# OpenBMB/VisRAG

Measured on AMD Instinct MI355X. Metric: page-images embedded/sec (VisRAG-Ret encode, 448x448, bf16 MFMA) + queries/sec@top-10 over 100k-page index, higher is better.
Workload: dtype bf16; 1 GPU; VisRAG-Ret (SigLIP-so400m 26 blk + resampler + MiniCPM-2B 40 layers) bf16 encode batch=32 page images 448x448 per GPU; index 100000 rows x 2304 sharded 1 way(s), 1000 queries top-10; batch_per_gpu=32, global_batch=32, parallelism=dp1 (pages sharded, no data-path collective)

## Files before the change

### include/visrag_hip.h

```cpp
#ifndef VISRAG_HIP_H
#define VISRAG_HIP_H

#include <stddef.h>
#include <stdint.h>

#ifdef __cplusplus
extern "C" {
#endif

#define VR_OK 0
#define VR_ERR_INVALID 1
#define VR_ERR_HIP 2
#define VR_ERR_STATE 3
#define VR_ERR_CAPACITY 4

#define VR_DTYPE_F32 0
#define VR_DTYPE_BF16 1

typedef struct vr_model_s* vr_model_t;
typedef struct vr_index_s* vr_index_t;

typedef struct vr_config {
    int32_t patch_size;
    int32_t vit_dim;
// ... 208 lines not shown

int vr_op_gemm(int device_id, const void* A, int32_t lda, const void* W, int32_t ldw,
               int32_t M, int32_t N, int32_t K, int32_t epilogue, const float* bias,
               const float* resid, float alpha, void* out, int32_t ldo,
               const int32_t* rope_pos, const float* rope_table, int32_t rope_cols,
               int32_t variant, void* stream);
typedef struct vr_gemm_extras {
    const int32_t* rowmap;
    const float* rowbias;
    int32_t rowbias_period, rowbias_ld, rowbias_cols;
    float col_scale;
    int32_t col_scale_n;
    int32_t ksplit;
    int64_t split_stride;
    const int32_t* m_dev;
    int32_t m_sub;
    int32_t raster_gm;
} vr_gemm_extras_t;
int vr_op_gemm_ex(int device_id, const void* A, int32_t lda, const void* W, int32_t ldw,
                  int32_t M, int32_t N, int32_t K, int32_t epilogue, const float* bias,
                  const float* resid, float alpha, void* out, int32_t ldo,
                  const int32_t* rope_pos, const float* rope_table, int32_t rope_cols,
                  int32_t variant, const vr_gemm_extras_t* extras, void* stream);
int vr_op_gemm_warm(int device_id, const void* A, int32_t lda, const void* W, int32_t ldw,
                    int32_t M, int32_t N, int32_t K, int32_t epilogue, const float* bias,
                    const float* resid, float alpha, void* out, int32_t ldo,
                    const int32_t* rope_pos, const float* rope_table, int32_t rope_cols,
                    int32_t variant, const vr_gemm_extras_t* extras, const void* warm, uint64_t warm_bytes, void* stream);
int vr_op_norm(int device_id, int32_t kind, const float* x, int32_t rows, int32_t dim,
               const float* weight, const float* bias, float eps, void* out, int32_t ldo,
               void* stream);
int vr_op_norm_ex(int device_id, int32_t kind, const float* x, int32_t rows, int32_t dim, int32_t ldx, const float* weight,
                  const float* bias, float eps, void* out, int32_t ldo, void* stream);

int vr_op_text_rmsnorm_split(int device_id, const float* x, int32_t rows, int32_t dim, const float* weight, float eps, void* hi,
                             void* lo, void* stream);
int vr_op_text_rope(int device_id, float* qkv, int32_t T, int32_t ld, int32_t rope_cols, const int32_t* pos, const float* table,
                    void* stream);
int vr_op_text_attention(int device_id, const float* qkv, int32_t ld, int32_t E, const int32_t* seq_offsets, int32_t B, int32_t T,
                         int32_t heads, float scale, float* out, void* stream);
int vr_op_text_swiglu_split(int device_id, const float* gu, int32_t T, int32_t ld_gu, int32_t I, int32_t ld_act, void* hi, void* lo,
                            void* stream);
int vr_op_embed_gather(int device_id, const int32_t* ids, int32_t T, const void* table, const void* table_lo, int32_t dim,
                       float scale, float* out, void* stream);
int vr_op_pool(int device_id, const float* h, const int32_t* seq_offsets, int32_t B, int32_t dim, const float* norm_w, float eps,
               float* out, float* tap, int32_t mode, void* stream);
int vr_op_convert(int device_id, int32_t kind, const void* in, void* out, void* out2, int64_t n, int64_t n_total, int32_t* aux,
                  void* stream);
int vr_op_planes_sum(int device_id, const float* parts, int32_t n_parts, int64_t stride, int32_t ldp, int32_t T, int32_t N,
                     float* out, int32_t ldo, float alpha, int32_t accumulate, void* stream);
int vr_op_patch_embed(int device_id, const void* const* imgs, int32_t n, int32_t H, int32_t W, int32_t P, const float* weight,
                      int32_t D, int32_t K, const float* bias, const float* pos, int32_t ld_pos, float* out, int32_t ldo,
                      void* stream);
int vr_op_attention(int device_id, const void* q, int32_t ldq, const void* k, int32_t ldk,
                    const void* v, int32_t ldv, void* out, int32_t ldo,
                    const int32_t* cu_q, const int32_t* cu_kv, int32_t B, int32_t heads,
                    int32_t head_dim, int32_t max_q, int32_t causal, int32_t q_shared,
                    float scale, void* stream);
typedef struct vr_attn_extras {
    int32_t kv_group;
    const int32_t* kv_end;
    const int32_t* q_in_rows;
    int32_t q_head_stride;
    int32_t q_prescaled;
    float* lse;
} vr_attn_extras_t;
int vr_op_attention_ex(int device_id, const void* q, int32_t ldq, const void* k, int32_t ldk,
                       const void* v, int32_t ldv, void* out, int32_t ldo,
                       const int32_t* cu_q, const int32_t* cu_kv, int32_t B, int32_t heads,
                       int32_t head_dim, int32_t max_q, int32_t causal, int32_t q_shared,
                       float scale, const vr_attn_extras_t* extras, void* stream);
int vr_op_attn_combine(int device_id, const void* part, const float* lse, int32_t S, const int32_t* S_dev, int32_t heads,
                       int32_t group, int32_t n_rows, void* out, int32_t ld_out, const void* W, int32_t ldw, int32_t M,
                       int32_t N, int32_t K, int32_t ksplit, int32_t planes, int32_t ldo, int64_t split_stride, void* stream);
int vr_op_gemm_skinny(int device_id, const void* A, int32_t lda, const void* W, int32_t ldw, int32_t M, int32_t N,
                      int32_t K, int32_t ksplit, const float* bias, int32_t swiglu, void* out, int32_t ldo,
                      int64_t split_stride, void* stream);
int vr_op_plane_sum(int device_id, int32_t kind, const float* parts, int32_t nsplit, int64_t split_stride, int32_t ldp,
                    int32_t rows, int32_t dim, float* x, int32_t ldx, float alpha, const float* weight, float eps,
                    void* out, int32_t ldo, void* stream);
int vr_op_chat_attention(int device_id, const void* q, const void* prompt, const void* tails, int32_t layers, int32_t l,
                         int32_t E, int32_t slots, int32_t max_len, int32_t rows, int32_t max_new, int32_t n,
                         const int32_t* step_row, const int32_t* step_slot, const int32_t* step_tail,
                         const int32_t* slot_plen, int32_t force_splits, void* att, void* stream);
int vr_op_chat_select(int device_id, int32_t mode, const float* logits, int32_t ld, int32_t V, const uint32_t* seen,
                      int32_t words, int32_t n_groups, const int32_t* group_offsets, const float* beam_scores, int32_t K,
                      int32_t kout, float repetition_penalty, float temperature, uint64_t seed, int32_t step,
                      float* out_scores, int32_t* out_tokens, int32_t* out_parents, void* stream);
int vr_op_chat_prompt_scatter(int device_id, const void* qkv, int32_t ld, int32_t E, int32_t B, const int32_t* seq_offsets,
                              const int32_t* slots, int32_t n_slots, int32_t max_len, void* kplane, void* vplane, void* stream);

int vr_op_gen_mrope_cache(int device_id, const void* src_bf16, const float* parts, int32_t n_parts, int64_t plane_stride,
                          const float* bias, int32_t ld, int32_t T, int32_t H, int32_t KV, const int32_t* pos3, int32_t pos_stride,
                          int32_t sec_t, int32_t sec_h, const float* inv_freq, void* q_out, int32_t ldq, void* k_cache, void* v_cache,
                          int32_t ld_cache, int32_t cache_row0, const int32_t* row0_dev, const int32_t* cache_rows, int32_t* cu_kv,
                          void* stream);
int vr_op_gen_rope2d(int device_id, void* qkv, int32_t ld, int32_t T, int32_t n_slots, int32_t hh, const int32_t* pos_h,
                     const int32_t* pos_w, int32_t sec_h, const float* freq, void* stream);
int vr_op_gen_sample(int device_id, const float* logits, int32_t vocab, uint32_t* seen, float repetition_penalty, float temperature,
                     uint64_t seed, int32_t step, int32_t* state, int32_t step_from_state, int32_t advance, int32_t* out_token,
                     void* stream);
int vr_op_gen_mark_seen(int device_id, const int32_t* ids, int32_t n, uint32_t* seen, int32_t vocab, void* stream);
int vr_op_gen_decode_begin(int device_id, int32_t* state, int32_t q_rows, void* stream);
int vr_op_gen_rows(int device_id, int32_t kind, const float* src, const int32_t* row_idx, int32_t n, int32_t dim, void* dst,
                   int32_t ld, const void* const* pages, const int32_t* page_w, int32_t n_pages, const int32_t* img, const int32_t* ph,
                   const int32_t* pw, int32_t P, int32_t tp, const float* mean3, const float* std3, void* stream);
// ... 6 lines not shown
```

### visrag_amd/_lib.py

```python
from __future__ import annotations

import ctypes as C
import os
from typing import Optional

_HERE = os.path.dirname(os.path.abspath(__file__))
LIB_PATH = os.path.join(_HERE, "libvisrag_hip.so")

VR_DTYPE_F32, VR_DTYPE_BF16 = 0, 1


class VRConfig(C.Structure):
    _fields_ = [
        ("patch_size", C.c_int32), ("vit_dim", C.c_int32), ("vit_depth", C.c_int32),
        ("vit_heads", C.c_int32), ("vit_hidden", C.c_int32), ("vit_pos_grid", C.c_int32),
        ("vit_ln_eps", C.c_float), ("query_num", C.c_int32), ("resampler_ln_eps", C.c_float),
        ("hidden_size", C.c_int32), ("num_layers", C.c_int32), ("num_heads", C.c_int32),
        ("intermediate_size", C.c_int32), ("vocab_size", C.c_int32), ("rms_norm_eps", C.c_float),
        ("rope_theta", C.c_float), ("scale_emb", C.c_float), ("residual_scale", C.c_float),
        ("max_images", C.c_int32), ("max_patches", C.c_int32), ("max_tokens", C.c_int32),
        ("max_seqs", C.c_int32), ("text_split_precision", C.c_int32),
    ]


# ... 65 lines not shown
    "vr_index_set_search_eps": (C.c_int, [_vp, _f32]),
    "vr_index_search_stats": (C.c_int, [_vp, C.POINTER(_i64), _i32]),
    "vr_index_error_model": (C.c_int, [_vp, C.POINTER(_f32)]),
    "vr_index_search_plan": (C.c_int, [_vp, _i32, C.POINTER(_i32)]),
    "vr_synth_pages": (C.c_int, [C.c_int, _vp, _i32, _i32, _i64, _i64, _vp]),
    "vr_streams_overlap": (C.c_int, [C.c_int, _vp, _vp, C.POINTER(C.c_int32)]),
    "vr_index_set_search_profile": (C.c_int, [_vp, _i32]),
    "vr_index_get_search_profile": (C.c_int, [_vp, C.POINTER(C.c_double), C.POINTER(_i64)]),
    "vr_index_search_keys": (C.c_int, [_vp, _vp, _i32, _i32, _i64, _vp, _i32, _vp]),
    "vr_index_set_groups": (C.c_int, [_vp, C.POINTER(_i64), _i64]),
    "vr_index_search_groups": (C.c_int, [_vp, _vp, _i32, _i32, _vp, _vp, _vp, _i32, _vp]),
    "vr_index_group_search_stats": (C.c_int, [_vp, C.POINTER(_i64), _i32]),
    "vr_index_set_filters": (C.c_int, [_vp, _vp, _i32, _i32, _vp]),
    "vr_index_search_filtered": (C.c_int, [_vp, _vp, _i32, _i32, _vp, _vp, _vp, _i32, _vp]),
    "vr_index_filter_search_stats": (C.c_int, [_vp, C.POINTER(_i64), _i32]),
    "vr_index_search_range": (C.c_int, [_vp, _vp, _i32, _vp, _vp, _i64, _vp, C.POINTER(_i64), _i32, _vp]),
    "vr_index_range_results": (C.c_int, [_vp, _vp, _vp, _i64, _i32, _vp]),
    "vr_index_range_search_stats": (C.c_int, [_vp, C.POINTER(_i64), _i32]),
    "vr_index_rank_rows": (C.c_int, [_vp, _vp, _i32, _vp, _vp, _vp, _vp, _vp, _i32, _vp]),
    "vr_index_count_range": (C.c_int, [_vp, _vp, _i32, _vp, _vp, _i32, _vp, _vp, _i32, _vp]),
    "vr_index_rank_search_stats": (C.c_int, [_vp, C.POINTER(_i64), _i32]),
    "vr_index_search_window": (C.c_int, [_vp, _vp, _i32, _vp, _i32, _vp, _vp, _vp, _i32, _vp]),
    "vr_index_window_search_stats": (C.c_int, [_vp, C.POINTER(_i64), _i32]),
    "vr_index_search_groups_window": (C.c_int, [_vp, _vp, _i32, _vp, _i32, _vp, _vp, _vp, _vp, _i32, _vp]),
    "vr_index_group_window_search_stats": (C.c_int, [_vp, C.POINTER(_i64), _i32]),
    "vr_index_rank_groups": (C.c_int, [_vp, _vp, _i32, _vp, _vp, _vp, _vp, _vp, _vp, _i32, _vp]),
    "vr_index_count_groups_range": (C.c_int, [_vp, _vp, _i32, _vp, _vp, _i32, _vp, _vp, _i32, _vp]),
    "vr_index_group_rank_search_stats": (C.c_int, [_vp, C.POINTER(_i64), _i32]),
    "vr_index_search_multi": (C.c_int, [_vp, _vp, _i32, _vp, _i32, _i32, _i32, _vp, _vp, _vp, _vp, _i32, _vp]),
    "vr_index_multi_search_stats": (C.c_int, [_vp, C.POINTER(_i64), _i32]),
    "vr_index_search_diverse": (C.c_int, [_vp, _vp, _i32, _i32, _i32, _f32, _vp, _vp, _vp, _i32, _vp]),
    "vr_index_remove": (C.c_int, [_vp, C.POINTER(_i64), _i64, C.POINTER(_i64), _vp]),
    "vr_index_update": (C.c_int, [_vp, C.POINTER(_i64), _vp, _i64, _i32, _vp]),
    "vr_index_get_rows": (C.c_int, [_vp, C.POINTER(_i64), _i64, _vp, _vp, _i32, _vp]),
    "vr_topk_merge_keys": (C.c_int, [C.c_int, _vp, _i32, _i32, _i32, _vp, _vp, _vp]),
    "vr_resize_bicubic": (C.c_int, [C.c_int, _vp, _i32, _i32, _i32, _vp, _i32, _i32, _vp]),
    "vr_op_gemm": (C.c_int, [C.c_int, _vp, _i32, _vp, _i32, _i32, _i32, _i32, _i32, _vp, _vp, _f32,
                             _vp, _i32, _vp, _vp, _i32, _i32, _vp]),
    "vr_op_gemm_ex": (C.c_int, [C.c_int, _vp, _i32, _vp, _i32, _i32, _i32, _i32, _i32, _vp, _vp, _f32,
                                _vp, _i32, _vp, _vp, _i32, _i32, C.POINTER(VRGemmExtras), _vp]),
    "vr_op_gemm_warm": (C.c_int, [C.c_int, _vp, _i32, _vp, _i32, _i32, _i32, _i32, _i32, _vp, _vp, _f32,
                                  _vp, _i32, _vp, _vp, _i32, _i32, C.POINTER(VRGemmExtras), _vp, C.c_uint64, _vp]),
    "vr_op_norm": (C.c_int, [C.c_int, _i32, _vp, _i32, _i32, _vp, _vp, _f32, _vp, _i32, _vp]),
    "vr_op_norm_ex": (C.c_int, [C.c_int, _i32, _vp, _i32, _i32, _i32, _vp, _vp, _f32, _vp, _i32, _vp]),
    "vr_op_text_rmsnorm_split": (C.c_int, [C.c_int, _vp, _i32, _i32, _vp, _f32, _vp, _vp, _vp]),
    "vr_op_text_rope": (C.c_int, [C.c_int, _vp, _i32, _i32, _i32, _vp, _vp, _vp]),
    "vr_op_text_attention": (C.c_int, [C.c_int, _vp, _i32, _i32, _vp, _i32, _i32, _i32, _f32, _vp, _vp]),
    "vr_op_text_swiglu_split": (C.c_int, [C.c_int, _vp, _i32, _i32, _i32, _i32, _vp, _vp, _vp]),
    "vr_op_embed_gather": (C.c_int, [C.c_int, _vp, _i32, _vp, _vp, _i32, _f32, _vp, _vp]),
    "vr_op_pool": (C.c_int, [C.c_int, _vp, _vp, _i32, _i32, _vp, _f32, _vp, _vp, _i32, _vp]),
    "vr_op_convert": (C.c_int, [C.c_int, _i32, _vp, _vp, _vp, _i64, _i64, _vp, _vp]),
    "vr_op_planes_sum": (C.c_int, [C.c_int, _vp, _i32, _i64, _i32, _i32, _i32, _vp, _i32, _f32, _i32, _vp]),
    "vr_op_patch_embed": (C.c_int, [C.c_int, C.POINTER(_vp), _i32, _i32, _i32, _i32, _vp, _i32, _i32, _vp, _vp, _i32, _vp, _i32, _vp]),
    "vr_op_attention": (C.c_int, [C.c_int, _vp, _i32, _vp, _i32, _vp, _i32, _vp, _i32, _vp, _vp, _i32,
                                  _i32, _i32, _i32, _i32, _i32, _f32, _vp]),
    "vr_op_attention_ex": (C.c_int, [C.c_int, _vp, _i32, _vp, _i32, _vp, _i32, _vp, _i32, _vp, _vp, _i32,
                                     _i32, _i32, _i32, _i32, _i32, _f32, C.POINTER(VRAttnExtras), _vp]),
    "vr_op_attn_combine": (C.c_int, [C.c_int, _vp, _vp, _i32, _vp, _i32, _i32, _i32, _vp, _i32, _vp, _i32, _i32, _i32, _i32, _i32,
                                     _i32, _i32, _i64, _vp]),
    "vr_op_gemm_skinny": (C.c_int, [C.c_int, _vp, _i32, _vp, _i32, _i32, _i32, _i32, _i32, _vp, _i32, _vp, _i32, _i64, _vp]),
    "vr_op_plane_sum": (C.c_int, [C.c_int, _i32, _vp, _i32, _i64, _i32, _i32, _i32, _vp, _i32, _f32, _vp, _f32, _vp, _i32, _vp]),
    "vr_op_chat_attention": (C.c_int, [C.c_int, _vp, _vp, _vp, _i32, _i32, _i32, _i32, _i32, _i32, _i32, _i32, C.POINTER(_i32),
                                       C.POINTER(_i32), C.POINTER(_i32), C.POINTER(_i32), _i32, _vp, _vp]),
    "vr_op_chat_select": (C.c_int, [C.c_int, _i32, _vp, _i32, _i32, _vp, _i32, _i32, C.POINTER(_i32), C.POINTER(_f32), _i32, _i32,
                                    _f32, _f32, C.c_uint64, _i32, C.POINTER(_f32), C.POINTER(_i32), C.POINTER(_i32), _vp]),
    "vr_op_chat_prompt_scatter": (C.c_int, [C.c_int, _vp, _i32, _i32, _i32, C.POINTER(_i32), C.POINTER(_i32), _i32, _i32, _vp, _vp, _vp]),
    "vr_op_gen_mrope_cache": (C.c_int, [C.c_int, _vp, _vp, _i32, _i64, _vp, _i32, _i32, _i32, _i32, _vp, _i32, _i32, _i32, _vp, _vp, _i32,
                                        _vp, _vp, _i32, _i32, _vp, _vp, _vp, _vp]),
    "vr_op_gen_rope2d": (C.c_int, [C.c_int, _vp, _i32, _i32, _i32, _i32, _vp, _vp, _i32, _vp, _vp]),
    "vr_op_gen_sample": (C.c_int, [C.c_int, _vp, _i32, _vp, _f32, _f32, C.c_uint64, _i32, _vp, _i32, _i32, C.POINTER(_i32), _vp]),
    "vr_op_gen_mark_seen": (C.c_int, [C.c_int, _vp, _i32, _vp, _i32, _vp]),
    "vr_op_gen_decode_begin": (C.c_int, [C.c_int, _vp, _i32, _vp]),
    "vr_op_gen_rows": (C.c_int, [C.c_int, _i32, _vp, _vp, _i32, _i32, _vp, _i32, C.POINTER(_vp), C.POINTER(_i32), _i32, _vp, _vp, _vp,
                                 _i32, _i32, C.POINTER(_f32), C.POINTER(_f32), _vp]),
    "vr_chat_create": (C.c_int, [_vp, C.POINTER(VRChatConfig), C.POINTER(_vp)]),
    "vr_chat_destroy": (C.c_int, [_vp]),
    "vr_chat_load_head": (C.c_int, [_vp, _vp, C.POINTER(_i64), _i32, _i32, _i32]),
    "vr_chat_prefill": (C.c_int, [_vp, _i32, _i32, C.POINTER(_vp), C.POINTER(_i32), _i32, _i32, C.POINTER(_i32), _i32,
                                  C.POINTER(_i32), _vp]),
    "vr_chat_prefill_batch": (C.c_int, [_vp, _i32, C.POINTER(_i32), C.POINTER(_i32), C.POINTER(_vp), C.POINTER(_i32), _i32, _i32,
                                        C.POINTER(_i32), C.POINTER(_i32), C.POINTER(_i32), _vp]),
    "vr_chat_step": (C.c_int, [_vp, _i32, C.POINTER(_i32), C.POINTER(_i32), C.POINTER(_i32), _vp]),
    "vr_chat_select": (C.c_int, [_vp, _i32, _i32, C.POINTER(_i32), C.POINTER(_i32), C.POINTER(_f32), _i32, _f32, _f32, _i32,
                                 C.c_uint64, _i32, C.POINTER(_f32), C.POINTER(_i32), C.POINTER(_i32), _vp]),
    "vr_chat_reorder": (C.c_int, [_vp, _i32, C.POINTER(_i32), C.POINTER(_i32), _vp]),
    "vr_chat_logits": (C.c_int, [_vp, _i32, _vp, _vp]),
    "vr_chat_row_len": (C.c_int, [_vp, _i32, C.POINTER(_i32), C.POINTER(_i32)]),
}
GEN_SIGNATURES = {
    "vg_create": (C.c_int, [C.c_int, C.POINTER(VGConfig), C.POINTER(_vp)]),
    "vg_destroy": (C.c_int, [_vp]),
    "vg_load_weight": (C.c_int, [_vp, C.c_char_p, _vp, C.POINTER(_i64), _i32, _i32, _i32]),
    "vg_finalize": (C.c_int, [_vp]),
    "vg_prefill": (C.c_int, [_vp, _vp, _i32, _vp, _vp, _i32, _vp, _vp]),
    "vg_sample": (C.c_int, [_vp, _f32, _f32, C.c_uint64, _i32, C.POINTER(_i32), _vp]),
    "vg_decode": (C.c_int, [_vp, _i32, C.POINTER(_i32), _vp]),
    "vg_logits": (C.c_int, [_vp, _vp, _vp]),
    "vg_select": (C.c_int, [_vp, _i32]),
    "vg_decode_batch": (C.c_int, [_vp, _i32, C.POINTER(_i32), C.POINTER(_i32), C.POINTER(_i32), _vp]),
    "vg_sample_batch": (C.c_int, [_vp, _i32, C.POINTER(_i32), _f32, _f32, C.c_uint64, _i32, C.POINTER(_i32), _vp]),
    "vg_cache_len": (C.c_int, [_vp, C.POINTER(_i32)]),
    "vg_run_begin": (C.c_int, [_vp, _i32, _f32, _f32, C.c_uint64, _i32, _vp]),
    "vg_run_step": (C.c_int, [_vp]),
    "vg_run_token": (C.c_int, [_vp, _i32, C.POINTER(_i32)]),
    "vg_run_end": (C.c_int, [_vp]),
    "vg_vision_create": (C.c_int, [_vp, C.POINTER(VGVisionConfig)]),
# ... 44 lines not shown
```

### visrag_amd/csrc/encode.hip

```cpp
#include <hip/hip_runtime.h>

#include <algorithm>
#include <cmath>
#include <cstring>
#include <vector>

#include "model.h"

static int run_vision_group(vr_model_s* m, const uint8_t* const* dev_imgs_hostarray, int n, int H, int W,
                            const int32_t* rowmap_host , bool first_group, hipStream_t s) {
    const vr_config_t& c = m->c;
    const int P = c.patch_size, gh = H / P, gw = W / P, N = gh * gw;
    const int D = m->D, Dp = m->Dp, E = m->E, Q = m->Q;
    const int M = n * N;
    GridTables* g = nullptr;
    VRCHK(get_grid(m, gh, gw, &g));

    HIPCHK(hipMemcpyAsync(m->w_imgptr.p, dev_imgs_hostarray, (size_t)n * 8, hipMemcpyHostToDevice, s));
    int* cu = (int*)arena_take(m, (size_t)2 * (n + 1) * 4);
    for (int i = 0; i <= n; ++i) { cu[i] = i * N; cu[n + 1 + i] = i * Q; }
    HIPCHK(hipMemcpyAsync(m->w_cu.p, cu, (size_t)2 * (n + 1) * 4, hipMemcpyHostToDevice, s));
    HIPCHK(hipMemcpyAsync(m->w_rowmap.p, rowmap_host, (size_t)n * Q * 4, hipMemcpyHostToDevice, s));
    const int* cu_tok = m->w_cu.as<int>();
    const int* cu_qry = m->w_cu.as<int>() + (n + 1);

    float* h = m->w_hvit.as<float>();
    {
        GemmArgs a = gemm_args(nullptr, 0, m->patch, M, h, Dp);
        a.rowbias = g->vit_pos.as<float>(); a.rowbias_period = N; a.rowbias_ld = Dp; a.rowbias_cols = Dp;
        HIPCHK(launch_patch_embed((const uint8_t* const*)m->w_imgptr.p, n, H, W, P, a, m->Kpe, s));
    }
    if (first_group) VRCHK(tap_store(m, "vit_embed", h, N, D, Dp, false, s));
    const int ldqkv = pad128(3 * D);
    const int vit_hd = c.vit_dim / c.vit_heads;
    const int vit_qscale_n = D % 64 == 0 ? D : 0;
    const float vit_qscale = (1.0f / sqrtf((float)vit_hd)) * 1.44269504088896340736f;
    for (int l = 0; l < c.vit_depth; ++l) {
        const VitBlock& b = m->blocks[l];
        HIPCHK(launch_layernorm(h, M, D, Dp, b.n1w.v.as<float>(), b.n1b.v.as<float>(), c.vit_ln_eps, m->w_xn.p, Dp, s));
        VRCHK(prof_begin(m, VR_PROF_VIT_QKV, s));
        {
            GemmArgs a = gemm_args(m->w_xn.p, Dp, b.qkv, M, m->w_qkv.p, ldqkv);
            a.col_scale = vit_qscale; a.col_scale_n = vit_qscale_n;
            HIPCHK(launch_gemm(a, EPI_BF16, GEMM_VARIANT_AUTO, s));
        }
        VRCHK(prof_end(m, VR_PROF_VIT_QKV, 2.0 * M * D * 3 * D, s));
        {
            AttnArgs a{};
            a.q = m->w_qkv.p; a.ldq = ldqkv;
            a.k = (const char*)m->w_qkv.p + (size_t)D * 2; a.ldk = ldqkv;
            a.v = (const char*)m->w_qkv.p + (size_t)2 * D * 2; a.ldv = ldqkv;
            a.out = m->w_att.p; a.ldo = Dp; a.cu_q = cu_tok; a.cu_kv = cu_tok; a.B = n; a.heads = c.vit_heads;
            a.head_dim = vit_hd; a.max_q = N; a.causal = 0; a.q_shared = 0; a.scale = 1.0f / sqrtf((float)vit_hd); a.q_prescaled = vit_qscale_n > 0;
            VRCHK(prof_begin(m, VR_PROF_VIT_ATTN, s));
            HIPCHK(launch_attention(a, s));
            VRCHK(prof_end(m, VR_PROF_VIT_ATTN, 4.0 * n * (double)N * N * D, s));
        }
        VRCHK(prof_begin(m, VR_PROF_VIT_PROJ, s));
        {
            GemmArgs a = gemm_args(m->w_att.p, Dp, b.proj, M, h, Dp); a.resid = h;
            HIPCHK(launch_gemm(a, EPI_RESID, GEMM_VARIANT_AUTO, s));
        }
        VRCHK(prof_end(m, VR_PROF_VIT_PROJ, 2.0 * M * D * D, s));
        HIPCHK(launch_layernorm(h, M, D, Dp, b.n2w.v.as<float>(), b.n2b.v.as<float>(), c.vit_ln_eps, m->w_xn.p, Dp, s));
        VRCHK(prof_begin(m, VR_PROF_VIT_FC1, s));
        { GemmArgs a = gemm_args(m->w_xn.p, Dp, b.fc1, M, m->w_mlp.p, m->Fp); HIPCHK(launch_gemm(a, EPI_GELU, GEMM_VARIANT_AUTO, s)); }
        VRCHK(prof_end(m, VR_PROF_VIT_FC1, 2.0 * M * D * m->F, s));
        VRCHK(prof_begin(m, VR_PROF_VIT_FC2, s));
        {
            GemmArgs a = gemm_args(m->w_mlp.p, m->Fp, b.fc2, M, h, Dp); a.resid = h;
            HIPCHK(launch_gemm(a, EPI_RESID, GEMM_VARIANT_AUTO, s));
        }
        VRCHK(prof_end(m, VR_PROF_VIT_FC2, 2.0 * M * D * m->F, s));
        if (l == 0 && first_group) VRCHK(tap_store(m, "vit_block0", h, N, D, Dp, false, s));
    }
    HIPCHK(launch_layernorm(h, M, D, Dp, m->vit_nw.v.as<float>(), m->vit_nb.v.as<float>(), c.vit_ln_eps, m->w_xn.p, Dp, s));
    if (first_group) VRCHK(tap_store(m, "vit_out", m->w_xn.p, N, D, Dp, true, s));

    VRCHK(prof_begin(m, VR_PROF_RESAMPLER, s));
    { GemmArgs a = gemm_args(m->w_xn.p, Dp, m->r_kvproj, M, m->w_kv32.p, E); HIPCHK(launch_gemm(a, EPI_F32, GEMM_VARIANT_AUTO, s)); }
    HIPCHK(launch_layernorm(m->w_kv32.as<float>(), M, E, E, m->r_lnkv_w.v.as<float>(), m->r_lnkv_b.v.as<float>(),
                            c.resampler_ln_eps, m->w_xkv.p, E, s));
    {
// ... 377 lines not shown
```

### visrag_amd/csrc/kernels.h

```cpp
#pragma once
#include <hip/hip_runtime.h>
#include <stdint.h>

#include "gemm_warm.h"

namespace vr {

enum GemmEpilogue { EPI_BF16 = 0, EPI_GELU = 1, EPI_F32 = 2, EPI_RESID = 3, EPI_SWIGLU = 4, EPI_ROPE = 5 };
enum GemmVariant { GEMM_VARIANT_GLDS = 0, GEMM_VARIANT_AUTO = 3, GEMM_VARIANT_192 = 7, GEMM_VARIANT_256IL = 9, GEMM_VARIANT_256W = 12,
                   GEMM_VARIANT_192W = 13, GEMM_VARIANT_128W_192 = 14, GEMM_VARIANT_128W_256 = 15 };

struct GemmArgs {
    const void* A; int lda;
    const void* W; int ldw;
    int M, N, K;
    const float* bias;
    const float* resid;
    float alpha;
    void* out; int ldo;
    const int* rowmap;
    const float* rowbias;
    int rowbias_period, rowbias_ld, rowbias_cols;
    const int* rope_pos;
    const float* rope_table;
// ... 82 lines not shown
hipError_t launch_chat_select(const ChatSel& sel, int mode, const float* logits, int ld, int V, const unsigned* seen, int words, float pen,
                              float temperature, int K, int kout, unsigned long long seed, unsigned step, float* lse,
                              unsigned long long* part, float* o_score, int* o_tok, int* o_par, hipStream_t s);

constexpr int GEN_ATT_SPLITS = 16;
struct GenState {
    int token;
    int pos[3];
    int len;
    int step;
    int splits;
    int pad;
    int cu_q[GEN_ATT_SPLITS + 1], cu_kv[GEN_ATT_SPLITS + 1];
};
struct KvSplit { int splits, chunk; };
__host__ __device__ inline KvSplit gen_kv_split(int L) {
    int splits = min(GEN_ATT_SPLITS, max(1, (L + 127) / 128));
    const int chunk = ((L + splits - 1) / splits + 63) / 64 * 64;
    splits = (L + chunk - 1) / chunk;
    return KvSplit{splits, chunk};
}
struct GenBatch {
    int token[16];
    int pos[3][16];
    int cache_row[16];
    int splits[16];
    int cu_q[16 * GEN_ATT_SPLITS + 1];
    int kv_lo[16 * GEN_ATT_SPLITS], kv_hi[16 * GEN_ATT_SPLITS];
    int q_in[16 * GEN_ATT_SPLITS];
    int sampled[16];
};
hipError_t launch_decode_begin(GenState* st, int q_rows, hipStream_t s);
hipError_t launch_mrope_cache(const void* src_bf16, const float* parts, int n_parts, size_t plane_stride, const float* bias,
                              int ld, int T, int H, int KV, const int* pos3, int pos_stride, int sec_t, int sec_h,
                              const float* inv_freq, void* q_out, int ldq, void* k_cache, void* v_cache, int ld_cache,
                              int cache_row0, int* cu_kv, hipStream_t s, const int* row0_dev = nullptr,
                              const int* cache_rows = nullptr);
hipError_t launch_rope2d_table(const int* pos_h, const int* pos_w, int T, int sec_h, const float* freq, void* cs, hipStream_t s);
hipError_t launch_rope2d_inplace(void* qkv, int ld, int T, int n_slots, int hh, const void* cs, hipStream_t s);
hipError_t launch_mark_seen(const int* ids, int n, unsigned* seen, int vocab, hipStream_t s);
hipError_t launch_sample(const float* logits, int vocab, unsigned* seen, float penalty, float temperature,
                         unsigned long long seed, unsigned step, int* token_out, unsigned long long* scratch64, hipStream_t s,
                         GenState* st = nullptr, int step_from_state = 0, int advance = 0);
hipError_t launch_scatter_rows(const float* src, const int* row_idx, int n, int dim, float* dst, int ld, hipStream_t s);
hipError_t launch_gather_rows_bf16(const float* src, const int* row_idx, int n, int dim, void* dst, int ld, hipStream_t s);
hipError_t launch_patch_rows_u8(const uint8_t* const* pages, const int* page_w, const int* img, const int* ph, const int* pw, int n,
                                int P, int tp, const float* mean3, const float* std3, void* dst, int ld, hipStream_t s);
hipError_t launch_attn_combine(const void* part, const float* lse, int S, int heads, int group, void* out, hipStream_t s,
                               const int* S_dev = nullptr,
                               int n_rows = 1, int ld_out = 0);

hipError_t launch_patch_embed(const uint8_t* const* imgs, int n_imgs, int H, int W, int P, const GemmArgs& g, int Kreal,
                              hipStream_t s);
hipError_t launch_embed_gather(const int* ids, int T, const void* table, int dim, float scale,
                               float* out, hipStream_t s);
hipError_t launch_pool(const float* h, const int* seq_offsets, int B, int dim, const float* norm_w,
                       float eps, float* out, float* tap_hidden, hipStream_t s, int mode = 0);
hipError_t launch_f32_to_bf16(const float* in, void* out, size_t n, hipStream_t s);
hipError_t launch_f32_to_bf16_pad(const float* in, void* out, size_t n, size_t n_total, hipStream_t s,
                                  int* zero_word = nullptr);
hipError_t launch_split_bf16(const float* in, void* hi, void* lo, size_t n, hipStream_t s);
hipError_t launch_iota_pos(const int* seq_offsets, int B, int* pos, hipStream_t s);
hipError_t launch_any_nonzero16(const void* p, size_t n, int* flag, hipStream_t s);

hipError_t launch_rmsnorm_split(const float* x, int rows, int dim, const float* w, float eps, void* hi, void* lo, hipStream_t s);
hipError_t launch_rope_f32(float* qkv, int T, int ld, int rope_cols, const int* pos, const float* table, hipStream_t s);
hipError_t launch_attn_f32(const float* qkv, int ld, int E, const int* seq_of, const int* seq_offsets, int T, int heads,
                           float scale, float* out, hipStream_t s);
hipError_t launch_swiglu_split(const float* gu, int T, int ld_gu, int I, int ld_act, void* hi, void* lo, hipStream_t s);
hipError_t launch_embed_gather_hp(const int* ids, int T, const void* table_hi, const void* table_lo, int dim, float scale,
                                  float* out, hipStream_t s);
hipError_t launch_seq_of(const int* seq_offsets, int B, int* seq_of, hipStream_t s);
hipError_t launch_planes_sum(const float* parts, int n_parts, size_t stride, int ldp, int T, int N, float* out, int ldo, float alpha,
                             bool accumulate, hipStream_t s);

hipError_t launch_synth_pages(uint8_t* out, int n, int size, long long seed, long long first, hipStream_t s);

}
#include <vector>
namespace vr {
int resize_coeffs(int in_size, int out_size, std::vector<int>& bounds, std::vector<int>& kk);
hipError_t launch_resize_h(const uint8_t* in, int in_w, int rows, uint8_t* out, int out_w, const int* bounds,
                           const int* kk, int ksize, hipStream_t s);
hipError_t launch_resize_v(const uint8_t* in, int w, uint8_t* out, int out_h, const int* bounds, const int* kk,
                           int ksize, hipStream_t s);

struct SearchArgs {
    const void* index_bf16;
    const float* index_f32;
    int64_t n_docs;
    int dim;
    const void* q_bf16;
    int convert_q;
    const float* q_f32;
    int nq, k;
    float* cand_scores; int* cand_ids; int n_chunks;
    float* out_scores; int64_t* out_ids;
    float* thr_init;
    int pre_own_chunks;
    float* thr_cert;
    unsigned long long* cand_keys;
    float* score_rows; size_t ld_scores;
    int exact_follows;
    int* huge_seen;
    const float* thr_used;
    float eps_rel;
// ... 195 lines not shown
```

### visrag_amd/csrc/ops.hip

```cpp
#include <hip/hip_runtime.h>

#include <algorithm>
#include <chrono>
#include <map>
#include <tuple>
#include <vector>

#include "engine_common.h"

struct ResizeTab { DevBuf bounds, kk; int ksize = 0; };
static std::map<std::tuple<int, int, int>, ResizeTab> g_resize_tabs;

static int get_resize_tab(int dev, int in_size, int out_size, ResizeTab** out) {
    auto key = std::make_tuple(dev, in_size, out_size);
    auto it = g_resize_tabs.find(key);
    if (it == g_resize_tabs.end()) {
        std::vector<int> b, k;
        ResizeTab t;
        t.ksize = resize_coeffs(in_size, out_size, b, k);
        VRCHK(t.bounds.alloc(b.size() * 4));
        VRCHK(t.kk.alloc(k.size() * 4));
        HIPCHK(hipMemcpy(t.bounds.p, b.data(), b.size() * 4, hipMemcpyHostToDevice));
        HIPCHK(hipMemcpy(t.kk.p, k.data(), k.size() * 4, hipMemcpyHostToDevice));
        it = g_resize_tabs.emplace(key, std::move(t)).first;
// ... 380 lines not shown
    return VR_OK;
}

extern "C" int vr_op_text_swiglu_split(int device_id, const float* gu, int32_t T, int32_t ld_gu, int32_t I, int32_t ld_act, void* hi,
                                       void* lo, void* stream) {
    if (!gu || !hi || !lo) return fail(VR_ERR_INVALID, "NULL argument");
    VRCHK(set_dev(device_id));
    HIPCHK(launch_swiglu_split(gu, T, ld_gu, I, ld_act, hi, lo, (hipStream_t)stream));
    return VR_OK;
}

extern "C" int vr_op_embed_gather(int device_id, const int32_t* ids, int32_t T, const void* table, const void* table_lo, int32_t dim,
                                  float scale, float* out, void* stream) {
    if (!ids || !table || !out) return fail(VR_ERR_INVALID, "NULL argument");
    VRCHK(set_dev(device_id));
    if (!table_lo) HIPCHK(launch_embed_gather(ids, T, table, dim, scale, out, (hipStream_t)stream));
    else HIPCHK(launch_embed_gather_hp(ids, T, table, table_lo, dim, scale, out, (hipStream_t)stream));
    return VR_OK;
}

extern "C" int vr_op_pool(int device_id, const float* h, const int32_t* seq_offsets, int32_t B, int32_t dim, const float* norm_w,
                          float eps, float* out, float* tap, int32_t mode, void* stream) {
    if (!h || !seq_offsets || !norm_w || !out) return fail(VR_ERR_INVALID, "NULL argument");
    VRCHK(set_dev(device_id));
    HIPCHK(launch_pool(h, seq_offsets, B, dim, norm_w, eps, out, tap, (hipStream_t)stream, mode));
    return VR_OK;
}

extern "C" int vr_op_convert(int device_id, int32_t kind, const void* in, void* out, void* out2, int64_t n, int64_t n_total,
                             int32_t* aux, void* stream) {
    if (kind < 0 || kind > 5) return fail(VR_ERR_INVALID, "kind %d: 0 f32->bf16, 1 f32->bf16 + zero pad, 2 hi/lo split, 3 any non-zero, 4 positions, 5 sequence of a token", kind);
    if (!in || (kind != 3 && !out) || (kind == 2 && !out2) || (kind == 3 && !aux)) return fail(VR_ERR_INVALID, "NULL argument");
    VRCHK(set_dev(device_id));
    hipStream_t s = (hipStream_t)stream;
    switch (kind) {
        case 0: HIPCHK(launch_f32_to_bf16((const float*)in, out, (size_t)n, s)); break;
        case 1: HIPCHK(launch_f32_to_bf16_pad((const float*)in, out, (size_t)n, (size_t)n_total, s, aux)); break;
        case 2: HIPCHK(launch_split_bf16((const float*)in, out, out2, (size_t)n, s)); break;
        case 3: HIPCHK(launch_any_nonzero16(in, (size_t)n, aux, s)); break;
        case 4: HIPCHK(launch_iota_pos((const int*)in, (int)n, (int*)out, s)); break;
        default: HIPCHK(launch_seq_of((const int*)in, (int)n, (int*)out, s)); break;
    }
    return VR_OK;
}

extern "C" int vr_op_planes_sum(int device_id, const float* parts, int32_t n_parts, int64_t stride, int32_t ldp, int32_t T, int32_t N,
                                float* out, int32_t ldo, float alpha, int32_t accumulate, void* stream) {
    if (!parts || !out) return fail(VR_ERR_INVALID, "NULL argument");
    VRCHK(set_dev(device_id));
    HIPCHK(launch_planes_sum(parts, n_parts, (size_t)stride, ldp, T, N, out, ldo, alpha, accumulate != 0, (hipStream_t)stream));
    return VR_OK;
}

extern "C" int vr_op_patch_embed(int device_id, const void* const* imgs, int32_t n, int32_t H, int32_t W, int32_t P, const float* weight,
                                 int32_t D, int32_t K, const float* bias, const float* pos, int32_t ld_pos, float* out, int32_t ldo,
                                 void* stream) {
    if (!imgs || !weight || !bias || !pos || !out) return fail(VR_ERR_INVALID, "NULL argument");
    for (int i = 0; i < n; ++i)
        if (!imgs[i]) return fail(VR_ERR_INVALID, "NULL argument");
    VRCHK(set_dev(device_id));
    hipStream_t s = (hipStream_t)stream;
    const int Kreal = 3 * P * P, patches = P > 0 ? (H / P) * (W / P) : 0;
    DevBuf wp, ptrs;
    VRCHK(wp.alloc((size_t)pad256(D > 0 ? D : 1) * (size_t)std::max(std::max(K, Kreal), 1) * 2));
    VRCHK(ptrs.alloc((size_t)(n > 0 ? n : 1) * sizeof(void*)));
    HIPCHK(launch_pack_patch_weight(weight, 0, D, P, wp.p, K, s));
    if (n > 0) HIPCHK(hipMemcpyAsync(ptrs.p, imgs, (size_t)n * sizeof(void*), hipMemcpyHostToDevice, s));
    GemmArgs a{};
    a.W = wp.p; a.ldw = K; a.M = n * patches; a.N = D; a.K = K; a.bias = bias; a.out = out; a.ldo = ldo; a.alpha = 1.0f;
    a.rowbias = pos; a.rowbias_period = patches; a.rowbias_ld = ld_pos; a.rowbias_cols = D;
    const hipError_t e = launch_patch_embed((const uint8_t* const*)ptrs.p, n, H, W, P, a, Kreal, s);
    HIPCHK(hipStreamSynchronize(s));
    if (e != hipSuccess) return fail(VR_ERR_HIP, "launch_patch_embed(...) failed: %s", hipGetErrorString(e));
    return VR_OK;
}

extern "C" int vr_op_gen_mrope_cache(int device_id, const void* src_bf16, const float* parts, int32_t n_parts, int64_t plane_stride,
                                     const float* bias, int32_t ld, int32_t T, int32_t H, int32_t KV, const int32_t* pos3,
                                     int32_t pos_stride, int32_t sec_t, int32_t sec_h, const float* inv_freq, void* q_out, int32_t ldq,
                                     void* k_cache, void* v_cache, int32_t ld_cache, int32_t cache_row0, const int32_t* row0_dev,
                                     const int32_t* cache_rows, int32_t* cu_kv, void* stream) {
    if ((!src_bf16 && !parts) || !pos3 || !inv_freq || !q_out || !k_cache || !v_cache) return fail(VR_ERR_INVALID, "NULL argument");
    if (T < 1 || H < 1 || KV < 1 || (parts && n_parts < 1)) return fail(VR_ERR_INVALID, "need T, H, KV >= 1 (and n_parts >= 1 with planes)");
    VRCHK(set_dev(device_id));
    HIPCHK(launch_mrope_cache(parts ? nullptr : src_bf16, parts, n_parts, (size_t)plane_stride, bias, ld, T, H, KV, pos3, pos_stride,
                              sec_t, sec_h, inv_freq, q_out, ldq, k_cache, v_cache, ld_cache, cache_row0, cu_kv, (hipStream_t)stream,
                              row0_dev, cache_rows));
    return VR_OK;
}

extern "C" int vr_op_gen_rope2d(int device_id, void* qkv, int32_t ld, int32_t T, int32_t n_slots, int32_t hh, const int32_t* pos_h,
                                const int32_t* pos_w, int32_t sec_h, const float* freq, void* stream) {
    if (!qkv || !pos_h || !pos_w || !freq) return fail(VR_ERR_INVALID, "NULL argument");
    if (T < 1 || n_slots < 1) return fail(VR_ERR_INVALID, "need T, n_slots >= 1");
    VRCHK(set_dev(device_id));
    hipStream_t s = (hipStream_t)stream;
    DevBuf cs;
    VRCHK(cs.alloc((size_t)T * 64 * 8));
    hipError_t e = launch_rope2d_table(pos_h, pos_w, T, sec_h, freq, cs.p, s);
    if (e == hipSuccess) e = launch_rope2d_inplace(qkv, ld, T, n_slots, hh, cs.p, s);
    HIPCHK(hipStreamSynchronize(s));
    if (e != hipSuccess) return fail(VR_ERR_HIP, "launch_rope2d_table / launch_rope2d_inplace(...) failed: %s", hipGetErrorString(e));
    return VR_OK;
}

static_assert(sizeof(GenState) == 42 * 4 && GEN_ATT_SPLITS == 16, "vr_op_gen_sample / vr_op_gen_decode_begin document 42 words");
static std::map<int, DevBuf> g_gen_op_scratch;

extern "C" int vr_op_gen_sample(int device_id, const float* logits, int32_t vocab, uint32_t* seen, float repetition_penalty,
                                float temperature, uint64_t seed, int32_t step, int32_t* state, int32_t step_from_state,
                                int32_t advance, int32_t* out_token, void* stream) {
    if (!logits || !seen || !out_token || ((step_from_state || advance) && !state)) return fail(VR_ERR_INVALID, "NULL argument");
    if (vocab < 1) return fail(VR_ERR_INVALID, "vocab must be positive");
    VRCHK(set_dev(device_id));
    hipStream_t s = (hipStream_t)stream;
    DevBuf& sc = g_gen_op_scratch[device_id];
    if (sc.bytes < 64 * 8 + 16) { HIPCHK(hipStreamSynchronize(s)); VRCHK(sc.reserve(64 * 8 + 16)); }
    int* tok = (int*)((char*)sc.p + 64 * 8);
    HIPCHK(launch_sample(logits, vocab, (unsigned*)seen, repetition_penalty, temperature, (unsigned long long)seed, (unsigned)step, tok,
                         sc.as<unsigned long long>(), s, (GenState*)state, step_from_state, advance));
    HIPCHK(hipMemcpyAsync(out_token, tok, 4, hipMemcpyDeviceToHost, s));
    HIPCHK(hipStreamSynchronize(s));
    return VR_OK;
}

extern "C" int vr_op_gen_mark_seen(int device_id, const int32_t* ids, int32_t n, uint32_t* seen, int32_t vocab, void* stream) {
// ... 46 lines not shown
```

### visrag_amd/csrc/patch_embed.hip

```cpp
#include "gemm_core.h"
#include "gemm_epilogue.h"
#include "kernels.h"

namespace vr {

struct PatchArgs {
    const uint8_t* const* imgs;
    int H, W, P, gw, N;
    GemmArgs g;
    int Kreal;
};

__global__ __launch_bounds__(256) void patch_embed_kernel(PatchArgs a) {
    extern __shared__ __attribute__((aligned(16))) char smem[];
    const GemmArgs& p = a.g;
    const int tiles_n = p.N / GEMM_BN;
    const int tiles_m = (p.M + GEMM_BM - 1) / GEMM_BM;
    const int t = xcd_remap(blockIdx.x, tiles_m * tiles_n);
    const int m0 = (t / tiles_n) * GEMM_BM, n0 = (t % tiles_n) * GEMM_BN;
    const int tid = threadIdx.x, lane = tid & 63, wave = tid >> 6;
    const int wm = wave >> 1, wn = wave & 1;
    const int rowbytes = a.W * 3, seg = a.P * 3;

    const int kc = tid & 7;
// ... 20 lines not shown
        }
    };
    auto write_tile = [&](char* tile, int k0) {
#pragma unroll
        for (int i = 0; i < 4; ++i) {
            const int row = (tid >> 3) + 32 * i;
            bf16x8 v;
#pragma unroll
            for (int e = 0; e < 8; ++e) {
                const float f = ((float)px8[i][e] / 255.0f - 0.5f) / 0.5f;
                v[e] = (rok[i] && k0 + kc * 8 + e < a.Kreal) ? f2bf(f) : (bf16_t)0.f;
            }
            *reinterpret_cast<bf16x8*>(tile + row * 128 + ((kc ^ (row & 7)) << 4)) = v;
        }
    };

    gemm_acc_t acc;
    gemm_zero(acc);
    const bf16_t* Wp = (const bf16_t*)p.W;
    const int nk = p.K / GEMM_BK;
    load_pixels(0);
    stage_glds(Wp, p.ldw, n0, 0, smem + GEMM_TILE_BYTES, wave, lane);
    write_tile(smem, 0);
    for (int kt = 0; kt < nk; ++kt) {
        char* cur = smem + (kt & 1) * 2 * GEMM_TILE_BYTES;
        char* nxt = smem + ((kt + 1) & 1) * 2 * GEMM_TILE_BYTES;
        __syncthreads();
        if (kt + 1 < nk) {
            load_pixels((kt + 1) * GEMM_BK);
            stage_glds(Wp, p.ldw, n0, (kt + 1) * GEMM_BK, nxt + GEMM_TILE_BYTES, wave, lane);
        }
        gemm_compute_tile(acc, cur, cur + GEMM_TILE_BYTES, wm, wn, lane);
        if (kt + 1 < nk) write_tile(nxt, (kt + 1) * GEMM_BK);
    }
#pragma unroll
    for (int i = 0; i < 4; ++i)
        gemm_epilogue_row<EPI_F32>(acc[i], p, m0 + wm * 64 + i * 16 + (lane & 15), n0 + wn * 64, lane >> 4);
}

hipError_t launch_patch_embed(const uint8_t* const* imgs, int n_imgs, int H, int W, int P, const GemmArgs& g, int Kreal,
                              hipStream_t s) {
    if (n_imgs <= 0) return hipSuccess;
    if (H % P || W % P || g.N % GEMM_BN || g.K % GEMM_BK || Kreal != 3 * P * P || Kreal > g.K || g.rowmap || g.ksplit > 1)
        return hipErrorInvalidValue;
    PatchArgs a{};
    a.imgs = imgs; a.H = H; a.W = W; a.P = P; a.gw = W / P; a.N = (H / P) * (W / P); a.g = g; a.Kreal = Kreal;
    const int tiles = (g.N / GEMM_BN) * ((g.M + GEMM_BM - 1) / GEMM_BM);
    static unsigned long long attr = 0;
    set_max_dynamic_lds((const void*)patch_embed_kernel, GEMM_SMEM_BYTES, attr);
    hipLaunchKernelGGL(patch_embed_kernel, dim3(tiles), dim3(256), GEMM_SMEM_BYTES, s, a);
    return hipGetLastError();
}

}
```

Measured before the change: 715.7 pages/s.

## Route patch embed through coalesced patch-row im2col plus the tuned GEMM

Adds a patch_rows kernel that stages contiguous image row segments into LDS with aligned 16-byte loads, normalizes the pixels through a LUT, and writes a padded bf16 im2col matrix. The encode path then runs the generic auto-selected GEMM on that matrix, borrowing the MLP weight buffer as scratch. This replaces the fused tile kernel's byte-granular gathered pixel loads. The cost is an extra write and read of the im2col matrix, and the route falls back to the fused kernel when the scratch buffer is too small.

Result: no change. 717.5 pages/s (median of 6 runs) (+0.3%).

```diff
diff --git a/include/visrag_hip.h b/include/visrag_hip.h
--- a/include/visrag_hip.h
+++ b/include/visrag_hip.h
@@ -284,6 +284,11 @@
 int vr_op_patch_embed(int device_id, const void* const* imgs, int32_t n, int32_t H, int32_t W, int32_t P, const float* weight,
                       int32_t D, int32_t K, const float* bias, const float* pos, int32_t ld_pos, float* out, int32_t ldo,
                       void* stream);
+int vr_op_patch_embed_ex(int device_id, const void* const* imgs, int32_t n, int32_t H, int32_t W, int32_t P, const float* weight,
+                         int32_t D, int32_t K, const float* bias, const float* pos, int32_t ld_pos, float* out, int32_t ldo,
+                         int32_t route, void* stream);
+int vr_op_patch_rows(int device_id, const void* const* imgs, int32_t n, int32_t H, int32_t W, int32_t P, void* out, int32_t Kp,
+                     void* stream);
 int vr_op_attention(int device_id, const void* q, int32_t ldq, const void* k, int32_t ldk,
                     const void* v, int32_t ldv, void* out, int32_t ldo,
                     const int32_t* cu_q, const int32_t* cu_kv, int32_t B, int32_t heads,
diff --git a/visrag_amd/_lib.py b/visrag_amd/_lib.py
--- a/visrag_amd/_lib.py
+++ b/visrag_amd/_lib.py
@@ -141,6 +141,8 @@
     "vr_op_convert": (C.c_int, [C.c_int, _i32, _vp, _vp, _vp, _i64, _i64, _vp, _vp]),
     "vr_op_planes_sum": (C.c_int, [C.c_int, _vp, _i32, _i64, _i32, _i32, _i32, _vp, _i32, _f32, _i32, _vp]),
     "vr_op_patch_embed": (C.c_int, [C.c_int, C.POINTER(_vp), _i32, _i32, _i32, _i32, _vp, _i32, _i32, _vp, _vp, _i32, _vp, _i32, _vp]),
+    "vr_op_patch_embed_ex": (C.c_int, [C.c_int, C.POINTER(_vp), _i32, _i32, _i32, _i32, _vp, _i32, _i32, _vp, _vp, _i32, _vp, _i32, _i32, _vp]),
+    "vr_op_patch_rows": (C.c_int, [C.c_int, C.POINTER(_vp), _i32, _i32, _i32, _i32, _vp, _i32, _vp]),
     "vr_op_attention": (C.c_int, [C.c_int, _vp, _i32, _vp, _i32, _vp, _i32, _vp, _i32, _vp, _vp, _i32,
                                   _i32, _i32, _i32, _i32, _i32, _f32, _vp]),
     "vr_op_attention_ex": (C.c_int, [C.c_int, _vp, _i32, _vp, _i32, _vp, _i32, _vp, _i32, _vp, _vp, _i32,
diff --git a/visrag_amd/csrc/encode.hip b/visrag_amd/csrc/encode.hip
--- a/visrag_amd/csrc/encode.hip
+++ b/visrag_amd/csrc/encode.hip
@@ -28,7 +28,7 @@
     {
         GemmArgs a = gemm_args(nullptr, 0, m->patch, M, h, Dp);
         a.rowbias = g->vit_pos.as<float>(); a.rowbias_period = N; a.rowbias_ld = Dp; a.rowbias_cols = Dp;
-        HIPCHK(launch_patch_embed((const uint8_t* const*)m->w_imgptr.p, n, H, W, P, a, m->Kpe, s));
+        HIPCHK(launch_patch_embed_routed((const uint8_t* const*)m->w_imgptr.p, n, H, W, P, a, m->Kpe, m->w_mlp.p, m->w_mlp.bytes, 0, s));
     }
     if (first_group) VRCHK(tap_store(m, "vit_embed", h, N, D, Dp, false, s));
     const int ldqkv = pad128(3 * D);
diff --git a/visrag_amd/csrc/kernels.h b/visrag_amd/csrc/kernels.h
--- a/visrag_amd/csrc/kernels.h
+++ b/visrag_amd/csrc/kernels.h
@@ -158,6 +158,10 @@
 
 hipError_t launch_patch_embed(const uint8_t* const* imgs, int n_imgs, int H, int W, int P, const GemmArgs& g, int Kreal,
                               hipStream_t s);
+hipError_t launch_patch_rows(const uint8_t* const* imgs, int n_imgs, int H, int W, int P, int Kreal, void* out, int Kp, hipStream_t s);
+bool patch_rows_route_fits(int n_imgs, int H, int W, int P, const GemmArgs& g, int Kreal, size_t scratch_bytes);
+hipError_t launch_patch_embed_routed(const uint8_t* const* imgs, int n_imgs, int H, int W, int P, const GemmArgs& g, int Kreal,
+                                     void* scratch, size_t scratch_bytes, int route, hipStream_t s);
 hipError_t launch_embed_gather(const int* ids, int T, const void* table, int dim, float scale,
                                float* out, hipStream_t s);
 hipError_t launch_pool(const float* h, const int* seq_offsets, int B, int dim, const float* norm_w,
diff --git a/visrag_amd/csrc/ops.hip b/visrag_amd/csrc/ops.hip
--- a/visrag_amd/csrc/ops.hip
+++ b/visrag_amd/csrc/ops.hip
@@ -456,26 +456,58 @@
     return VR_OK;
 }
 
+static int op_patch_embed_route(int device_id, const void* const* imgs, int32_t n, int32_t H, int32_t W, int32_t P, const float* weight,
+                                int32_t D, int32_t K, const float* bias, const float* pos, int32_t ld_pos, float* out, int32_t ldo,
+                                int32_t route, void* stream) {
+    if (!imgs || !weight || !bias || !pos || !out) return fail(VR_ERR_INVALID, "NULL argument");
+    if (route < 0 || route > 2) return fail(VR_ERR_INVALID, "route %d: 0 as the engine chooses, 1 tile kernel, 2 patch rows + GEMM", route);
+    for (int i = 0; i < n; ++i)
+        if (!imgs[i]) return fail(VR_ERR_INVALID, "NULL argument");
+    VRCHK(set_dev(device_id));
+    hipStream_t s = (hipStream_t)stream;
+    const int Kreal = 3 * P * P, patches = P > 0 ? (H / P) * (W / P) : 0;
+    DevBuf wp, ptrs, rows;
+    VRCHK(wp.alloc((size_t)pad256(D > 0 ? D : 1) * (size_t)std::max(std::max(K, Kreal), 1) * 2));
+    VRCHK(ptrs.alloc((size_t)(n > 0 ? n : 1) * sizeof(void*)));
+    GemmArgs a{};
+    a.W = wp.p; a.ldw = K; a.M = n * patches; a.N = D; a.K = K; a.bias = bias; a.out = out; a.ldo = ldo; a.alpha = 1.0f;
+    a.rowbias = pos; a.rowbias_period = patches; a.rowbias_ld = ld_pos; a.rowbias_cols = D;
+    const size_t rows_bytes = a.M > 0 && K > 0 ? (size_t)pad256(a.M) * (size_t)K * 2 : 0;
+    if (route != 1 && rows_bytes && patch_rows_route_fits(n, H, W, P, a, Kreal, rows_bytes)) VRCHK(rows.alloc(rows_bytes));
+    HIPCHK(launch_pack_patch_weight(weight, 0, D, P, wp.p, K, s));
+    if (n > 0) HIPCHK(hipMemcpyAsync(ptrs.p, imgs, (size_t)n * sizeof(void*), hipMemcpyHostToDevice, s));
+    const hipError_t e = launch_patch_embed_routed((const uint8_t* const*)ptrs.p, n, H, W, P, a, Kreal, rows.p, rows.p ? rows_bytes : 0, route, s);
+    HIPCHK(hipStreamSynchronize(s));
+    if (e != hipSuccess)
+        return fail(VR_ERR_HIP, "%s(...) failed: %s", route == 2 ? "launch_patch_embed_routed" : "launch_patch_embed", hipGetErrorString(e));
+    return VR_OK;
+}
+
 extern "C" int vr_op_patch_embed(int device_id, const void* const* imgs, int32_t n, int32_t H, int32_t W, int32_t P, const float* weight,
                                  int32_t D, int32_t K, const float* bias, const float* pos, int32_t ld_pos, float* out, int32_t ldo,
                                  void* stream) {
-    if (!imgs || !weight || !bias || !pos || !out) return fail(VR_ERR_INVALID, "NULL argument");
+    return op_patch_embed_route(device_id, imgs, n, H, W, P, weight, D, K, bias, pos, ld_pos, out, ldo, 0, stream);
+}
+
+extern "C" int vr_op_patch_embed_ex(int device_id, const void* const* imgs, int32_t n, int32_t H, int32_t W, int32_t P, const float* weight,
+                                    int32_t D, int32_t K, const float* bias, const float* pos, int32_t ld_pos, float* out, int32_t ldo,
+                                    int32_t route, void* stream) {
+    return op_patch_embed_route(device_id, imgs, n, H, W, P, weight, D, K, bias, pos, ld_pos, out, ldo, route, stream);
+}
+
+extern "C" int vr_op_patch_rows(int device_id, const void* const* imgs, int32_t n, int32_t H, int32_t W, int32_t P, void* out, int32_t Kp,
+                                void* stream) {
+    if (!imgs || !out) return fail(VR_ERR_INVALID, "NULL argument");
     for (int i = 0; i < n; ++i)
         if (!imgs[i]) return fail(VR_ERR_INVALID, "NULL argument");
     VRCHK(set_dev(device_id));
     hipStream_t s = (hipStream_t)stream;
-    const int Kreal = 3 * P * P, patches = P > 0 ? (H / P) * (W / P) : 0;
-    DevBuf wp, ptrs;
-    VRCHK(wp.alloc((size_t)pad256(D > 0 ? D : 1) * (size_t)std::max(std::max(K, Kreal), 1) * 2));
+    DevBuf ptrs;
     VRCHK(ptrs.alloc((size_t)(n > 0 ? n : 1) * sizeof(void*)));
-    HIPCHK(launch_pack_patch_weight(weight, 0, D, P, wp.p, K, s));
     if (n > 0) HIPCHK(hipMemcpyAsync(ptrs.p, imgs, (size_t)n * sizeof(void*), hipMemcpyHostToDevice, s));
-    GemmArgs a{};
-    a.W = wp.p; a.ldw = K; a.M = n * patches; a.N = D; a.K = K; a.bias = bias; a.out = out; a.ldo = ldo; a.alpha = 1.0f;
-    a.rowbias = pos; a.rowbias_period = patches; a.rowbias_ld = ld_pos; a.rowbias_cols = D;
-    const hipError_t e = launch_patch_embed((const uint8_t* const*)ptrs.p, n, H, W, P, a, Kreal, s);
-    HIPCHK(hipStreamSynchronize(s));
-    if (e != hipSuccess) return fail(VR_ERR_HIP, "launch_patch_embed(...) failed: %s", hipGetErrorString(e));
+    const hipError_t e = launch_patch_rows((const uint8_t* const*)ptrs.p, n, H, W, P, 3 * P * P, out, Kp, s);
+    HIPCHK(hipStreamSynchronize(s));
+    if (e != hipSuccess) return fail(VR_ERR_HIP, "launch_patch_rows(...) failed: %s", hipGetErrorString(e));
     return VR_OK;
 }
 
diff --git a/visrag_amd/csrc/patch_embed.hip b/visrag_amd/csrc/patch_embed.hip
--- a/visrag_amd/csrc/patch_embed.hip
+++ b/visrag_amd/csrc/patch_embed.hip
@@ -96,4 +96,130 @@
     return hipGetLastError();
 }
 
-}
+constexpr int PATCH_ROWS_RUN = 64;
+constexpr int PATCH_ROWS_LUT = 512;
+constexpr int PATCH_ROWS_PAD = 64;
+
+struct PatchRowsArgs {
+    const uint8_t* const* imgs;
+    bf16_t* out;
+    int W, P, gh, gw;
+    int nblk, run;
+    int cpr, pitch;
+    int Kp, Kreal, M, Mp;
+    int runs;
+};
+
+__global__ __launch_bounds__(256) void patch_rows_kernel(PatchRowsArgs a) {
+    extern __shared__ __attribute__((aligned(16))) char smem[];
+    const int tid = threadIdx.x;
+    const int chunks = a.Kp >> 3;
+    if ((int)blockIdx.x >= a.runs) {
+        const int r0 = a.M + ((int)blockIdx.x - a.runs) * PATCH_ROWS_PAD;
+        const int rows = min(PATCH_ROWS_PAD, a.Mp - r0);
+        bf16x8 z;
+#pragma unroll
+        for (int e = 0; e < 8; ++e) z[e] = (bf16_t)0.f;
+        for (int i = tid; i < rows * chunks; i += 256) *reinterpret_cast<bf16x8*>(a.out + (size_t)r0 * a.Kp + (size_t)i * 8) = z;
+        return;
+    }
+    bf16_t* lut = reinterpret_cast<bf16_t*>(smem);
+    uint8_t* pix = reinterpret_cast<uint8_t*>(smem) + PATCH_ROWS_LUT;
+    lut[tid] = f2bf(((float)tid / 255.0f - 0.5f) / 0.5f);
+
+    const int blk = blockIdx.x % a.nblk, t = blockIdx.x / a.nblk;
+    const int py = t % a.gh, img = t / a.gh;
+    const int px0 = blk * a.run, nb = min(a.run, a.gw - px0);
+    const int seg = a.P * 3, rowbytes = a.W * 3, len = nb * seg;
+    const uint8_t* base = a.imgs[img] + (size_t)(py * a.P) * rowbytes + px0 * seg;
+    const unsigned base_lo = (unsigned)(uintptr_t)base;
+
+    for (int idx = tid; idx < a.P * a.cpr; idx += 256) {
+        const int ky = idx / a.cpr, c = idx - ky * a.cpr;
+        const uint8_t* src = base + (size_t)ky * rowbytes;
+        const int lo = c * 16 - (int)((base_lo + (unsigned)(ky * rowbytes)) & 15u);
+        if (lo >= len) continue;
+        uint8_t* dst = pix + ky * a.pitch + c * 16;
+        if (lo >= 0 && lo + 16 <= len) {
+            *reinterpret_cast<uint4*>(dst) = *reinterpret_cast<const uint4*>(src + lo);
+        } else {
+            for (int e = 0; e < 16; ++e)
+                if (lo + e >= 0 && lo + e < len) dst[e] = src[lo + e];
+        }
+    }
+    __syncthreads();
+
+    const size_t m0 = ((size_t)img * a.gh + py) * a.gw + px0;
+    for (int idx = tid; idx < nb * chunks; idx += 256) {
+        const int p = idx / chunks, kc = idx - p * chunks;
+        int k = kc * 8;
+        int ky = k / seg, off = k - ky * seg;
+        bf16x8 v;
+#pragma unroll
+        for (int e = 0; e < 8; ++e, ++k) {
+            if (k < a.Kreal) {
+                const int head = (int)((base_lo + (unsigned)(ky * rowbytes)) & 15u);
+                v[e] = lut[pix[ky * a.pitch + head + p * seg + off]];
+            } else {
+                v[e] = (bf16_t)0.f;
+            }
+            if (++off == seg) { off = 0; ++ky; }
+        }
+        *reinterpret_cast<bf16x8*>(a.out + (m0 + p) * a.Kp + kc * 8) = v;
+    }
+}
+
+static bool patch_rows_geometry(int H, int W, int P, int Kreal, int Kp, PatchRowsArgs& a) {
+    if (P < 1 || H < P || W < P || H % P || W % P || Kreal != 3 * P * P || Kreal > Kp || Kp % 8) return false;
+    a.W = W; a.P = P; a.gh = H / P; a.gw = W / P; a.Kp = Kp; a.Kreal = Kreal;
+    a.run = min(a.gw, PATCH_ROWS_RUN);
+    a.nblk = (a.gw + a.run - 1) / a.run;
+    a.cpr = (a.run * 3 * P + 30) / 16;
+    a.pitch = a.cpr * 16;
+    return PATCH_ROWS_LUT + (size_t)P * a.pitch <= 64 * 1024;
+}
+
+hipError_t launch_patch_rows(const uint8_t* const* imgs, int n_imgs, int H, int W, int P, int Kreal, void* out, int Kp, hipStream_t s) {
+    if (n_imgs <= 0) return hipSuccess;
+    PatchRowsArgs a{};
+    if (!patch_rows_geometry(H, W, P, Kreal, Kp, a)) return hipErrorInvalidValue;
+    const long long M = (long long)n_imgs * a.gh * a.gw;
+    if (M > (1ll << 30)) return hipErrorInvalidValue;
+    a.imgs = imgs; a.out = (bf16_t*)out; a.M = (int)M; a.Mp = (int)((M + 255) / 256 * 256);
+    a.runs = n_imgs * a.gh * a.nblk;
+    const int lds = PATCH_ROWS_LUT + P * a.pitch;
+    const int grid = a.runs + (a.Mp - a.M + PATCH_ROWS_PAD - 1) / PATCH_ROWS_PAD;
+    static unsigned long long attr = 0;
+    set_max_dynamic_lds((const void*)patch_rows_kernel, 64 * 1024, attr);
+    hipLaunchKernelGGL(patch_rows_kernel, dim3(grid), dim3(256), lds, s, a);
+    return hipGetLastError();
+}
+
+bool patch_rows_route_fits(int n_imgs, int H, int W, int P, const GemmArgs& g, int Kreal, size_t scratch_bytes) {
+    PatchRowsArgs a{};
+    if (n_imgs <= 0 || g.N % GEMM_BN || g.K % GEMM_BK || g.rowmap || g.ksplit > 1 || !patch_rows_geometry(H, W, P, Kreal, g.K, a)) return false;
+    const long long M = (long long)n_imgs * a.gh * a.gw, Mp = (M + 255) / 256 * 256;
+    if (M != g.M || (unsigned long long)Mp * g.K * 2 > scratch_bytes) return false;
+    GemmArgs q = g;
+    q.lda = g.K;
+    const int v = gemm_auto_variant(q, EPI_F32);
+    if (gemm_args_refused(q, EPI_F32, v)) return false;
+    if ((v == GEMM_VARIANT_256W || v == GEMM_VARIANT_192W) && !gemm256w_fits(q, v == GEMM_VARIANT_192W ? 192 : 256)) return false;
+    return true;
+}
+
+hipError_t launch_patch_embed_routed(const uint8_t* const* imgs, int n_imgs, int H, int W, int P, const GemmArgs& g, int Kreal,
+                                     void* scratch, size_t scratch_bytes, int route, hipStream_t s) {
+    if (route < 0 || route > 2) return hipErrorInvalidValue;
+    if (n_imgs <= 0) return hipSuccess;
+    const bool fits = route != 1 && scratch && patch_rows_route_fits(n_imgs, H, W, P, g, Kreal, scratch_bytes);
+    if (route == 2 && !fits) return hipErrorInvalidValue;
+    if (!fits) return launch_patch_embed(imgs, n_imgs, H, W, P, g, Kreal, s);
+    hipError_t e = launch_patch_rows(imgs, n_imgs, H, W, P, Kreal, scratch, g.K, s);
+    if (e != hipSuccess) return e;
+    GemmArgs q = g;
+    q.A = scratch; q.lda = g.K;
+    return launch_gemm(q, EPI_F32, GEMM_VARIANT_AUTO, s);
+}
+
+}
```
